# LauraFJulia/TFT_vs_Fund

Measured on AMD Instinct MI355X. Metric: triplet-hypotheses/sec (linearTFT+R,t) at N=200 corresp., higher is better.
Workload: dtype f64; 1 GPU; configs[1]: batch of 10000 synthetic triplets x 200 correspondences, sigma=1px, linearTFT + R_t_from_TFT (LinearTFTPoseEstimation without Reconst), one batch per GPU; batch_per_gpu=10000, correspondences=200, streams=2 (consecutive batches alternate between streams and may overlap), gather=none (1 GPU), failed_triplets=0, warmup_steps_run=2560

## Files before the change

tft_vs_fund_amd/csrc/pose_common.h:

```cpp
#pragma once
#include "wave.h"
#include "small_la.h"
#include "wave_eig.h"
#include "row_eig.h"
#include "wave_qr.h"

namespace tff {

constexpr int FLAG_RECONST = 1;
constexpr int FLAG_JACOBI = 2;
constexpr int FLAG_STAGE_LDS = 4;
constexpr int FLAG_ONLY_RETRY = 8;
constexpr int FLAG_DBG_FP_HANDOVER = 64;
constexpr int FLAG_DBG_ADAPTIVE = 32;
constexpr int FLAG_XI_IN_LDS = 128;
constexpr int FLAG_GH_EXACT = 16;

constexpr int ST_OK = 0;
constexpr int ST_TOO_FEW = 1;
constexpr int ST_NONFINITE = 2;
constexpr int ST_NO_POSE = 3;
constexpr int ST_RETRY = 100;

constexpr int DBG_STRIDE = 128;
// ... 445 lines not shown
                L[r][j] = sv * inv[j];
            }
        }
        double z[3];
#pragma unroll
        for (int r = 2; r >= 0; --r) {
            double sum = -L[3][r];
#pragma unroll
            for (int k = r + 1; k < 3; ++k) sum -= L[k][r] * z[k];
            z[r] = sum * inv[r];
        }
        const double d1 = z[2], d2 = R3[0] * z[0] + R3[1] * z[1] + R3[2] * z[2] + R3[3];
        const double d4 = S33 + delta - (L[3][0] * L[3][0] + L[3][1] * L[3][1] + L[3][2] * L[3][2]);
        const double zz = z[0] * z[0] + z[1] * z[1] + z[2] * z[2];
        const double idet = (inv[0] * inv[1]) * (inv[0] * inv[1]) * (inv[2] * inv[2]);
        const double trs = tr3 + 3.0 * delta;
        const double e = trs * trs * idet;
        const double Gp = 4.0 * (1.0 + zz) - d4 * e;
        const double rhs = 2.0 * d4 * e + 2.5e-14 * trs * e * Gp;
        const double dmin2 = fmin(d1 * d1, d2 * d2);
        const bool certain = Gp > 0.0 && dmin2 * Gp * Gp > rhs * rhs * zz;
        all_certain = all_certain && certain;
        score += (int)sgn(d1) + (int)sgn(d2);
    }
    return 2 * wave_sum_i(score) + (wave_any(!all_certain) ? 1 : 0);
}
struct VoteCam { double PB[12], R3[4]; };
struct VoteFactor { double L[4][3], inv[3], d4, z[3], pfloor; };
template <bool KEEP = false, bool CERT = true>
__device__ __forceinline__ void vote_one(const double (&SA)[6], const VoteCam& cam, const double x2, const double y2, int& score, bool& all_certain,
                                         VoteFactor* keep = nullptr) {
    double b0[4], b1[4];
#pragma unroll
    for (int c = 0; c < 4; ++c) { b0[c] = y2 * cam.PB[8 + c] - cam.PB[4 + c]; b1[c] = cam.PB[c] - x2 * cam.PB[8 + c]; }
    double S[4][3];
#pragma unroll
    for (int r = 0; r < 4; ++r)
#pragma unroll
        for (int c = 0; c < 3; ++c) {
            if (c > r) continue;
            double v = b0[r] * b0[c] + b1[r] * b1[c];
            if (r < 3) v += SA[r * (r + 1) / 2 + c];
            S[r][c] = v;
        }
    const double S33 = b0[3] * b0[3] + b1[3] * b1[3];
    const double tr3 = S[0][0] + S[1][1] + S[2][2];
    const double delta = 1e-14 * (tr3 + S33), pfloor = 1e-3 * delta + 1e-300;
    double L[4][3], inv[3];
#pragma unroll
    for (int j = 0; j < 3; ++j) {
        double d = S[j][j] + delta;
#pragma unroll
        for (int k = 0; k < j; ++k) d -= L[j][k] * L[j][k];
        d = fmax(d, pfloor);
        inv[j] = rsqrt_pos(d);
#pragma unroll
        for (int r = j + 1; r < 4; ++r) {
            double sv = S[r][j];
#pragma unroll
            for (int k = 0; k < j; ++k) sv -= L[r][k] * L[j][k];
            L[r][j] = sv * inv[j];
        }
    }
    double z[3];
#pragma unroll
    for (int r = 2; r >= 0; --r) {
        double sum = -L[3][r];
#pragma unroll
        for (int k = r + 1; k < 3; ++k) sum -= L[k][r] * z[k];
        z[r] = sum * inv[r];
    }
    const double d4 = S33 + delta - (L[3][0] * L[3][0] + L[3][1] * L[3][1] + L[3][2] * L[3][2]);
    if constexpr (CERT) {
        const double d1 = z[2], d2 = cam.R3[0] * z[0] + cam.R3[1] * z[1] + cam.R3[2] * z[2] + cam.R3[3];
        const double zz = z[0] * z[0] + z[1] * z[1] + z[2] * z[2];
        const double idet = (inv[0] * inv[1]) * (inv[0] * inv[1]) * (inv[2] * inv[2]);
        const double trs = tr3 + 3.0 * delta;
        const double e = trs * trs * idet;
        const double Gp = 4.0 * (1.0 + zz) - d4 * e;
        const double rhs = 2.0 * d4 * e + 2.5e-14 * trs * e * Gp;
        const double dmin2 = fmin(d1 * d1, d2 * d2);
        const bool certain = Gp > 0.0 && dmin2 * Gp * Gp > rhs * rhs * zz;
        all_certain = all_certain && certain;
        score += (int)sgn(d1) + (int)sgn(d2);
    }
    if constexpr (KEEP) {
#pragma unroll
        for (int r = 0; r < 4; ++r)
#pragma unroll
            for (int c = 0; c < 3; ++c) keep->L[r][c] = (c < r) ? L[r][c] : 0.0;
#pragma unroll
        for (int c = 0; c < 3; ++c) { keep->inv[c] = inv[c]; keep->z[c] = z[c]; }
        keep->d4 = d4;
        keep->pfloor = pfloor;
    }
}
__device__ __forceinline__ bool dlt_from_vote(const VoteFactor& f, double (&X)[4]) {
    double L[4][4], inv[4];
#pragma unroll
    for (int r = 0; r < 4; ++r)
#pragma unroll
        for (int c = 0; c < 4; ++c) L[r][c] = (c < r) ? f.L[r][c] : 0.0;
    inv[0] = f.inv[0]; inv[1] = f.inv[1]; inv[2] = f.inv[2];
    inv[3] = rsqrt_pos(fmax(f.d4, f.pfloor));
    const double nn0 = 1.0 + (f.z[0] * f.z[0] + f.z[1] * f.z[1] + f.z[2] * f.z[2]);
    const double r0 = rsqrt(nn0);
    const bool fin = nn0 <= 1e300;
    X[0] = fin ? f.z[0] * r0 : 0.5; X[1] = fin ? f.z[1] * r0 : 0.5; X[2] = fin ? f.z[2] * r0 : 0.5; X[3] = fin ? r0 : 0.5;
    bool conv;
    chol_invit<4>(L, inv, X, 40, &conv);
    return conv;
}
template <bool CAM1_IN_REGISTERS>
__device__ __attribute__((noinline)) int tri_vote_fast2(PoseLds* w, const double* pts, int N, int view, const double* camB0, const double* Rt0,
                                                        const double* camB1, const double* Rt1) {
    const int lane = lane_id();
    double PA[12];
    VoteCam c0, c1r;
    load_uniform12(w->Pfin[0], PA);
    load_uniform12(camB0, c0.PB);
#pragma unroll
    for (int c = 0; c < 4; ++c) c0.R3[c] = wave_uniform(Rt0[8 + c]);
    if constexpr (CAM1_IN_REGISTERS) {
#pragma unroll
        for (int c = 0; c < 12; ++c) c1r.PB[c] = camB1[c];
#pragma unroll
        for (int c = 0; c < 4; ++c) c1r.R3[c] = Rt1[8 + c];
    }
    int score0 = 0, score1 = 0;
    bool certain0 = true, certain1 = true;
    Pt6 pnext = load_pt(pts, (lane < N) ? lane : 0);
#pragma unroll 1
    for (int i = lane; i < N; i += WAVE) {
        const Pt6 p = pnext;
        if (i + WAVE < N) pnext = load_pt(pts, i + WAVE);
        const double x1 = p.v[0], y1 = p.v[1], x2 = (view == 1) ? p.v[2] : p.v[4], y2 = (view == 1) ? p.v[3] : p.v[5];
        double a0[3], a1[3], SA[6];
#pragma unroll
        for (int c = 0; c < 3; ++c) { a0[c] = y1 * PA[8 + c] - PA[4 + c]; a1[c] = PA[c] - x1 * PA[8 + c]; }
#pragma unroll
        for (int r = 0; r < 3; ++r)
#pragma unroll
            for (int c = 0; c <= r; ++c) SA[r * (r + 1) / 2 + c] = a0[r] * a0[c] + a1[r] * a1[c];
        vote_one(SA, c0, x2, y2, score0, certain0);
        if constexpr (CAM1_IN_REGISTERS) {
            vote_one(SA, c1r, x2, y2, score1, certain1);
        } else {
            VoteCam c1;
            const double* pb = camB1 + opaque_int(0);
            const double* pr = Rt1 + opaque_int(0);
#pragma unroll
            for (int c = 0; c < 12; ++c) c1.PB[c] = pb[c];
#pragma unroll
            for (int c = 0; c < 4; ++c) c1.R3[c] = pr[8 + c];
            vote_one(SA, c1, x2, y2, score1, certain1);
        }
    }
    const int r0 = 2 * wave_sum_i(score0) + (wave_any(!certain0) ? 1 : 0), r1 = 2 * wave_sum_i(score1) + (wave_any(!certain1) ? 1 : 0);
    return (int)(((unsigned)r1 << 16) | ((unsigned)r0 & 0xffffu));
}
__device__ __attribute__((noinline)) int tri_vote_exact(PoseLds* w, const double* pts, int N, int view, const double* camB, const double* Rt) {
    const int lane = lane_id();
    typedef const double (&cam_ref)[12];
    cam_ref PA = *reinterpret_cast<const double(*)[12]>(w->Pfin[0]);
    cam_ref PB = *reinterpret_cast<const double(*)[12]>(camB);
    double R3[4];
#pragma unroll
// ... 243 lines not shown
```

tft_vs_fund_amd/csrc/small_la.h:

```cpp
#pragma once
#include "wave.h"

namespace tff {

struct Mat3 { double m[3][3]; };

__device__ __forceinline__ double sgn(double x) { return (x > 0.0) ? 1.0 : ((x < 0.0) ? -1.0 : 0.0); }

__device__ __forceinline__ Mat3 mat3_mul(const Mat3& a, const Mat3& b) {
    Mat3 c;
#pragma unroll
    for (int i = 0; i < 3; ++i)
#pragma unroll
        for (int j = 0; j < 3; ++j) c.m[i][j] = a.m[i][0] * b.m[0][j] + a.m[i][1] * b.m[1][j] + a.m[i][2] * b.m[2][j];
    return c;
}
__device__ __forceinline__ Mat3 mat3_T(const Mat3& a) {
    Mat3 c;
#pragma unroll
    for (int i = 0; i < 3; ++i)
#pragma unroll
        for (int j = 0; j < 3; ++j) c.m[i][j] = a.m[j][i];
    return c;
}
__device__ __forceinline__ double mat3_det(const Mat3& a) {
    return a.m[0][0] * (a.m[1][1] * a.m[2][2] - a.m[1][2] * a.m[2][1])
         - a.m[0][1] * (a.m[1][0] * a.m[2][2] - a.m[1][2] * a.m[2][0])
         + a.m[0][2] * (a.m[1][0] * a.m[2][1] - a.m[1][1] * a.m[2][0]);
}
__device__ __forceinline__ Mat3 mat3_inv(const Mat3& a) {
    Mat3 c;
    c.m[0][0] = a.m[1][1] * a.m[2][2] - a.m[1][2] * a.m[2][1];
    c.m[0][1] = a.m[0][2] * a.m[2][1] - a.m[0][1] * a.m[2][2];
    c.m[0][2] = a.m[0][1] * a.m[1][2] - a.m[0][2] * a.m[1][1];
    c.m[1][0] = a.m[1][2] * a.m[2][0] - a.m[1][0] * a.m[2][2];
    c.m[1][1] = a.m[0][0] * a.m[2][2] - a.m[0][2] * a.m[2][0];
    c.m[1][2] = a.m[0][2] * a.m[1][0] - a.m[0][0] * a.m[1][2];
    c.m[2][0] = a.m[1][0] * a.m[2][1] - a.m[1][1] * a.m[2][0];
    c.m[2][1] = a.m[0][1] * a.m[2][0] - a.m[0][0] * a.m[2][1];
    c.m[2][2] = a.m[0][0] * a.m[1][1] - a.m[0][1] * a.m[1][0];
    const double id = 1.0 / (a.m[0][0] * c.m[0][0] + a.m[0][1] * c.m[1][0] + a.m[0][2] * c.m[2][0]);
#pragma unroll
    for (int i = 0; i < 3; ++i)
#pragma unroll
        for (int j = 0; j < 3; ++j) c.m[i][j] *= id;
    return c;
}
__device__ __forceinline__ void cross3(const double* a, const double* b, double* c) {
    c[0] = a[1] * b[2] - a[2] * b[1];
    c[1] = a[2] * b[0] - a[0] * b[2];
    c[2] = a[0] * b[1] - a[1] * b[0];
}

__device__ __forceinline__ double det4(const double (&m)[4][4]) {
    const double s0 = m[0][0] * m[1][1] - m[1][0] * m[0][1], s1 = m[0][0] * m[1][2] - m[1][0] * m[0][2];
    const double s2 = m[0][0] * m[1][3] - m[1][0] * m[0][3], s3 = m[0][1] * m[1][2] - m[1][1] * m[0][2];
    const double s4 = m[0][1] * m[1][3] - m[1][1] * m[0][3], s5 = m[0][2] * m[1][3] - m[1][2] * m[0][3];
    const double c5 = m[2][2] * m[3][3] - m[3][2] * m[2][3], c4 = m[2][1] * m[3][3] - m[3][1] * m[2][3];
    const double c3 = m[2][1] * m[3][2] - m[3][1] * m[2][2], c2 = m[2][0] * m[3][3] - m[3][0] * m[2][3];
    const double c1 = m[2][0] * m[3][2] - m[3][0] * m[2][2], c0 = m[2][0] * m[3][1] - m[3][0] * m[2][1];
    return s0 * c5 - s1 * c4 + s2 * c3 + s3 * c2 - s4 * c1 + s5 * c0;
}

template <int n>
__device__ __forceinline__ int chol_invit(const double (&L)[n][n], const double (&inv)[n], double (&x)[n], const int maxit, bool* converged) {
    bool conv = false;
    double rprev2 = 1.0;
    int it = 0;
#pragma clang loop unroll(disable)
    for (; it < maxit;) {
        double y[n];
#pragma unroll
        for (int i = 0; i < n; ++i) {
            double s = x[i];
#pragma unroll
            for (int k = 0; k < i; ++k) s -= L[i][k] * y[k];
            y[i] = s * inv[i];
        }
#pragma unroll
        for (int i = n - 1; i >= 0; --i) {
            double s = y[i];
#pragma unroll
            for (int k = i + 1; k < n; ++k) s -= L[k][i] * y[k];
            y[i] = s * inv[i];
        }
        double nn = 0.0, dot = 0.0;
#pragma unroll
        for (int i = 0; i < n; ++i) { nn += y[i] * y[i]; dot += y[i] * x[i]; }
        const double rn = rsqrt(nn);
        const double sg = (dot < 0.0) ? -rn : rn;
// ... 401 lines not shown
```

tft_vs_fund_amd/csrc/tft_kernel.h:

```cpp
#pragma once
#include "pose_common.h"

namespace tff {

struct LinearTftArgs {
    const double* corresp;
    const double* calm;
    long calm_stride;
    long B;
    int N;
    int flags;
    double* Rt2;
    double* Rt3;
    double* T;
    double* reconst;
    int* iter;
    int* status;
    double* dbg;
    const int* sample_idx;
    double* init_p;
    double* init_x;
    double* spill;
    long spill_stride;
    int sample_ns;
    const double* pre;
    int* retry_list;
    int* retry_count;
    int* retry_zero;
    const long* offsets;
    const int* rlist;
    const int* rrange;
    int stage_upto;
};

constexpr int EIG_MAXIT = 300;
constexpr int RETRY_HINT_SHIFT = 28;
constexpr int RETRY_INDEX_MASK = (1 << RETRY_HINT_SHIFT) - 1;

__device__ __forceinline__ int ragged_n(const long* offsets, const long b) { return opaque_int(wave_uniform_i((int)(offsets[b + 1] - offsets[b]))); }
__device__ __forceinline__ int ragged_flags(const LinearTftArgs& a, const int n) {
    return opaque_int(n <= a.stage_upto ? (a.flags | FLAG_STAGE_LDS) : (a.flags & ~FLAG_STAGE_LDS));
}
template <bool RAGGED>
__device__ __forceinline__ void ragged_nan_outputs(const LinearTftArgs& a, const long b, const long rb, const int N) {
    if constexpr (RAGGED) wave_nan_outputs(a.Rt2 + b * 12, a.Rt3 + b * 12, a.T + b * 27, a.reconst ? a.reconst + 3 * rb : nullptr, 0, N);
    else wave_nan_outputs(a.Rt2, a.Rt3, a.T, a.reconst, b, N);
}

__device__ __forceinline__ void cvec(const double* a, const double* b, double (&c)[4]) {
    c[0] = a[0] * b[0] + a[1] * b[1];
    c[1] = -(a[0] * b[2] + a[2] * b[0]);
    c[2] = -(a[1] * b[2] + a[2] * b[1]);
    c[3] = a[2] * b[2];
}
__device__ __forceinline__ int hht_index(int i, int ip) {
    const int a = (i < ip) ? i : ip, b = (i < ip) ? ip : i;
    return (a == 0) ? b : ((a == 1) ? 2 + b : 5);
}
__device__ __forceinline__ double bilinear44(const double* M, const double (&c3)[4], const double (&c2)[4]) {
    double acc = 0.0;
#pragma unroll
    for (int p = 0; p < 4; ++p)
        acc += c3[p] * (M[4 * p] * c2[0] + M[4 * p + 1] * c2[1] + M[4 * p + 2] * c2[2] + M[4 * p + 3] * c2[3]);
    return acc;
}

__device__ inline void accumulate_moments(PoseLds* w, const double* pts, int N) {
    const int lane = lane_id();
    const double s1 = w->nrm[0], ox1 = w->nrm[1], oy1 = w->nrm[2];
    const double s2 = w->nrm[3], ox2 = w->nrm[4], oy2 = w->nrm[5];
    const double s3 = w->nrm[6], ox3 = w->nrm[7], oy3 = w->nrm[8];
#pragma unroll 1
    for (int pass = 0; pass < 3; ++pass) {
        double acc[32];
#pragma unroll
        for (int k = 0; k < 32; ++k) acc[k] = 0.0;
        for (int i = lane; i < N; i += WAVE) {
            const Pt6 p = load_pt(pts, i);
            const double x1 = s1 * p.v[0] + ox1, y1 = s1 * p.v[1] + oy1;
            const double x2 = s2 * p.v[2] + ox2, y2 = s2 * p.v[3] + oy2;
            const double x3 = s3 * p.v[4] + ox3, y3 = s3 * p.v[5] + oy3;
            const double q2[4] = {1.0, x2, y2, x2 * x2 + y2 * y2};
            const double q3[4] = {1.0, x3, y3, x3 * x3 + y3 * y3};
            const double pa = (pass == 0) ? x1 * x1 : ((pass == 1) ? x1 : y1);
            const double pb = (pass == 0) ? x1 * y1 : ((pass == 1) ? y1 * y1 : 1.0);
#pragma unroll
            for (int b = 0; b < 4; ++b)
#pragma unroll
                for (int c = 0; c < 4; ++c) {
                    const double wv = q3[b] * q2[c];
                    acc[4 * b + c] += pa * wv;
                    acc[16 + 4 * b + c] += pb * wv;
                }
        }
        const double tot = wave_reduce_scatter<32>(acc);
        if ((lane & 1) == 0) w->mom[32 * pass + reduce32_index(lane)] = tot;
    }
    wave_sync();
}

__device__ __forceinline__ void ctc_entry(int j, int jp, double& sign, int& idx) {
    const int a = (j < jp) ? j : jp, b = (j < jp) ? jp : j;
    if (b < 2) { sign = (a == b) ? 1.0 : 0.0; idx = 0; }
    else if (a < 2) { sign = -1.0; idx = 1 + a; }
    else { sign = 1.0; idx = 3; }
}
__device__ __forceinline__ void gram_row27(const double* mom, int r, double (&g)[27], double& diag) {
    const int i = r / 9, k = (r % 9) / 3, j = r % 3;
    double s2[3], s3[3];
    int i2[3], i3[3];
#pragma unroll
    for (int q = 0; q < 3; ++q) { ctc_entry(j, q, s2[q], i2[q]); ctc_entry(k, q, s3[q], i3[q]); }
#pragma unroll
    for (int ip = 0; ip < 3; ++ip) {
        const double* M = mom + 16 * hht_index(i, ip);
#pragma unroll
        for (int kp = 0; kp < 3; ++kp)
#pragma unroll
            for (int jp = 0; jp < 3; ++jp) g[jp + 3 * kp + 9 * ip] = s2[jp] * s3[kp] * M[4 * i3[kp] + i2[jp]];
    }
    diag = 0.0;
#pragma unroll
    for (int c = 0; c < 27; ++c) diag = (c == r) ? g[c] : diag;
}

__device__ __forceinline__ void frame_of(const double* e, double* Q) {
    const double a0 = fabs(e[0]), a1 = fabs(e[1]), a2 = fabs(e[2]);
    double ax[3] = {0.0, 0.0, 0.0};
    if (a0 <= a1 && a0 <= a2) ax[0] = 1.0; else if (a1 <= a2) ax[1] = 1.0; else ax[2] = 1.0;
    double q1[3], q2[3];
    cross3(e, ax, q1);
    const double n1 = rsqrt(q1[0] * q1[0] + q1[1] * q1[1] + q1[2] * q1[2]);
    q1[0] *= n1; q1[1] *= n1; q1[2] *= n1;
    cross3(e, q1, q2);
    const double n2 = rsqrt(q2[0] * q2[0] + q2[1] * q2[1] + q2[2] * q2[2]);
#pragma unroll
    for (int r = 0; r < 3; ++r) { Q[3 * r] = e[r]; Q[3 * r + 1] = q1[r]; Q[3 * r + 2] = q2[r] * n2; }
}

__device__ __forceinline__ void up_factors(const double* Q, int m, double (&a2)[3], double (&a3)[3]) {
    const int jj = (m < 3) ? 0 : m - 2, kk = (m < 3) ? m : 0;
#pragma unroll
    for (int q = 0; q < 3; ++q) { a2[q] = Q[3 * q + jj]; a3[q] = Q[9 + 3 * q + kk]; }
}

__device__ inline void tft_system_qr(const double* pts, const int N, const double* nrm, double* Rl) {
    const int lane = lane_id();
    for (int e = lane; e < 27 * 27; e += WAVE) Rl[e] = 0.0;
    wave_sync();
    const int col = (lane < 27) ? lane : 0, ci = col / 9, ck = (col % 9) / 3, cj = col % 3;
#pragma unroll 1
    for (int base = 0; base < N; base += 7) {
        double a[28];
#pragma unroll
        for (int q = 0; q < 7; ++q) {
            const int i = base + q;
            const Pt6 p = premap(load_pt(pts, (i < N) ? i : 0), nrm);
            const double h = (i < N && lane < 27) ? ((ci == 0) ? p.v[0] : (ci == 1) ? p.v[1] : 1.0) : 0.0;
            const double c2x = (cj == 0) ? 1.0 : (cj == 1) ? 0.0 : -p.v[2], c2y = (cj == 0) ? 0.0 : (cj == 1) ? 1.0 : -p.v[3];
            const double c3x = (ck == 0) ? 1.0 : (ck == 1) ? 0.0 : -p.v[4], c3y = (ck == 0) ? 0.0 : (ck == 1) ? 1.0 : -p.v[5];
            const double hx = h * c3x, hy = h * c3y;
            a[4 * q + 0] = hx * c2x; a[4 * q + 1] = hx * c2y; a[4 * q + 2] = hy * c2x; a[4 * q + 3] = hy * c2y;
        }
        wave_qr_cols_append<27, 28>(a, Rl);
    }
}

template <bool JAC, int G>
__device__ inline bool linear_tft_middle(PoseLds* w, JacobiLds* jw, const double* pts, int N, bool want_P, double* dbg, const int hint = 0) {
    static_assert(!JAC || G == 64, "the exact solver works on whole wavefronts");
    using Grp = Group<G>;
    const int lane = Grp::lane();
    const int wl = Grp::index() * G;
    int it1 = 0, it2 = 0;
    bool ok = true;
    {
        double x;
        if (JAC) {
            tft_system_qr(pts, N, w->nrm, jw->A);
            phase_stamp(dbg, 3, wl);
            double g[27];
            wave_qr_rows_from_lds<27>(jw->A, g);
            x = wave_qr_min_rsv<27>(g, jw->A, w->Lp, w->Lp, (hint & 1) ? 0 : EIG_MAXIT, &it1);
            if (it1 >= 1000) {
                if (lane < 27) w->t[lane] = x;
                wave_sync();
                tft_system_qr(pts, N, w->nrm, jw->A);
                x = (lane < 27) ? w->t[lane] : 0.0;
            }
            it1 += 10000;
        } else {
            double r2, risk;
            if constexpr (G == 64) {
                const int p = opaque_lane_int(lane & 15);
                const bool hi = p < 11;
                double ga[27], gb[27], g0[16], da, db;
                gram_row27(w->mom, p, ga, da);
                gram_row27(w->mom, hi ? 16 + p : 0, gb, db);
#pragma unroll
                for (int c = 0; c < 16; ++c) g0[c] = ga[c];
#pragma unroll
                for (int c = 0; c < 27; ++c) gb[c] = hi ? gb[c] : 0.0;
                phase_stamp(dbg, 3, wl);
                x = row_min_eigvec<27>(g0, gb, da, hi ? db : 0.0, w->Lp, EIG_MAXIT, &it1, &r2, false, 0.0, 0.0, &risk);
            } else {
                double g[27], diag;
                gram_row27(w->mom, (lane < 27) ? lane : 0, g, diag);
                phase_stamp(dbg, 3, wl);
                x = wave_min_eigvec_reg<27, G>(g, diag, w->Lp, EIG_MAXIT, &it1, &r2, false, 0.0, &risk);
            }
            ok = ok && eig_converged(r2) && risk == 0.0;
        }
        if (lane < 27) w->t[lane] = x;
        wave_sync();
    }
    if (dbg && lane < 27) dbg[lane] = w->t[lane];
    phase_stamp(dbg, 4, wl);
    ok = epipoles_from_tensor<G, JAC>(w->t, w->nullv, w->epi, false) && ok;
    phase_stamp(dbg, 5, wl);
    if (dbg && lane < 6) dbg[27 + lane] = w->epi[lane];
    if (lane == 0) frame_of(w->epi, w->Q);
    if (lane == 1) frame_of(w->epi + 3, w->Q + 9);
    wave_sync();
    if (JAC) {
        double* Bm = w->Lp;
        if (lane < 27) {
// ... 230 lines not shown
```

tft_vs_fund_amd/csrc/tft_rows_kernel.h:

```cpp
#pragma once
#include "tft_kernel.h"
#include "tft_moments_kernel.h"

namespace tff {

constexpr int ROW_TRIPLETS = 4;
constexpr int ROWL = 16;

struct RowRt {
    double T1[28];
    double T2[28];
    double nullv[18];
    double mats[28];
    double Ein[18];
    double cand[2][21];
    double P[4][12];
    double candRt[4][12];
    double Rt[2][12];
    double Pfin[3][12];
};
constexpr int ROW_OV_DOUBLES = 380;
static_assert(sizeof(RowRt) <= ROW_OV_DOUBLES * sizeof(double), "overlay");
struct RowLds {
    double mom[96];
    double nrm[9];
    double calm[27];
    double t[27];
    double epi[6];
    double Q[18];
    double tp[15];
    double pa[18];
    double ov[ROW_OV_DOUBLES];
};
constexpr int ROW_LDS_DOUBLES = (int)(sizeof(RowLds) / sizeof(double));
static_assert(ROW_LDS_DOUBLES % 2 == 0, "16-byte row stride");
inline size_t rows_lds_bytes() { return (size_t)ROW_TRIPLETS * sizeof(RowLds); }
inline unsigned rows_grid(long B) { const long g = (B + ROW_TRIPLETS - 1) / ROW_TRIPLETS; return (unsigned)(g > 0 ? g : 1); }

__device__ __forceinline__ int rows_p() { return lane_id() & 15; }

struct RowSrc { const double* pts; const int* idx; int ns; bool sampled; };
__device__ __forceinline__ Pt6 rows_load(const RowSrc& s, const int i) {
    if (s.sampled) {
        int k = s.idx[i];
        k = (k >= 0 && k < s.ns) ? k : 0;
        return load_pt(s.pts, k);
    }
    return load_pt(s.pts, i);
}

__device__ __forceinline__ void rows_stamp(double* dbg, const int slot) {
    if (dbg) {
        const long long t = shader_clock();
        if (rows_p() == 0) dbg[80 + slot] = (double)t;
    }
}


__device__ __forceinline__ void rows_centroids(const RowSrc& s, const int N, double (&c)[6]) {
    const int p = rows_p();
    double sm[6] = {0, 0, 0, 0, 0, 0};
#pragma unroll 1
    for (int i0 = 0; i0 < N; i0 += 4 * ROWL) {
        Pt6 q[4];
#pragma unroll
        for (int u = 0; u < 4; ++u) { const int i = i0 + ROWL * u + p; q[u] = rows_load(s, (i < N) ? i : 0); }
#pragma unroll
        for (int u = 0; u < 4; ++u) {
            const bool have = i0 + ROWL * u + p < N;
#pragma unroll
            for (int k = 0; k < 6; ++k) sm[k] += have ? q[u].v[k] : 0.0;
        }
    }
#pragma unroll
    for (int k = 0; k < 6; ++k) c[k] = row_sum16(sm[k]) / (double)N;
}

__device__ __forceinline__ void rows_distances_moments(const RowSrc& s, const int N, const double (&c)[6], double* nrm, double (&nr)[9], double* mom) {
    const int p = rows_p();
    const int slot = p >> 1;
    const bool odd = (p & 1) != 0;
    double acc[48];
#pragma unroll
    for (int k = 0; k < 48; ++k) acc[k] = 0.0;
    double dA = 0.0, dB = 0.0;
    auto body = [&](const Pt6& q, double& r2_out) {
        const double x1 = q.v[0] - c[0], y1 = q.v[1] - c[1];
        const double x2 = q.v[2] - c[2], y2 = q.v[3] - c[3];
        const double x3 = q.v[4] - c[4], y3 = q.v[5] - c[5];
        const double r1 = x1 * x1 + y1 * y1, r2 = x2 * x2 + y2 * y2, r3 = x3 * x3 + y3 * y3;
        dA += sqrt_nonneg(odd ? r3 : r1);
        r2_out = r2;
        const double q2[4] = {1.0, x2, y2, r2};
        const double q3[4] = {1.0, x3, y3, r3};
        const double pa = odd ? y1 * y1 : x1 * x1, pb = odd ? y1 : x1 * y1, pc = odd ? 1.0 : x1;
#pragma unroll
        for (int b = 0; b < 4; ++b)
#pragma unroll
            for (int cc = 0; cc < 4; ++cc) {
                const double wv = q3[b] * q2[cc];
                acc[4 * b + cc] += pa * wv;
                acc[16 + 4 * b + cc] += pb * wv;
                acc[32 + 4 * b + cc] += pc * wv;
            }
    };
    constexpr int STEP = ROWL / 2;
    Pt6 pe = rows_load(s, (slot < N) ? slot : 0);
    Pt6 po = rows_load(s, (slot + STEP < N) ? slot + STEP : 0);
#pragma unroll 1
    for (int i = slot; i < N; i += 2 * STEP) {
        const Pt6 q = pe;
        if (i + 2 * STEP < N) pe = rows_load(s, i + 2 * STEP);
        double r2a, r2b = 0.0;
        body(q, r2a);
        if (i + STEP < N) {
            const Pt6 r = po;
            if (i + 3 * STEP < N) po = rows_load(s, i + 3 * STEP);
            body(r, r2b);
        }
        dB += sqrt_nonneg(odd ? r2b : r2a);
    }
    const double d1 = row_sum16(odd ? 0.0 : dA), d3 = row_sum16(odd ? dA : 0.0), d2 = row_sum16(dB);
    const double r2c = sqrt(2.0);
    const double dd[3] = {d1, d2, d3};
#pragma unroll
    for (int v = 0; v < 3; ++v) {
        const double norm0 = dd[v] / (double)N;
        nr[3 * v + 0] = r2c / norm0;
        nr[3 * v + 1] = -r2c * c[2 * v] / norm0;
        nr[3 * v + 2] = -r2c * c[2 * v + 1] / norm0;
    }
    if (p < 9) {
        double mine = nr[0];
#pragma unroll
        for (int k = 1; k < 9; ++k) mine = (p == k) ? nr[k] : mine;
        nrm[p] = mine;
    }
#pragma unroll
    for (int i = 0; i < 24; ++i) acc[i] = halve_sum<8>(acc[i], acc[i + 24]);
#pragma unroll
    for (int i = 0; i < 12; ++i) acc[i] = halve_sum<4>(acc[i], acc[i + 12]);
#pragma unroll
    for (int i = 0; i < 6; ++i) acc[i] = halve_sum<2>(acc[i], acc[i + 6]);
    const int base = 6 * ((p >> 1) & 1) + 12 * ((p >> 2) & 1) + 24 * ((p >> 3) & 1);
    const double s1 = nr[0], s2 = nr[3], s3 = nr[6];
#pragma unroll
// ... 80 lines not shown
            if (r2 <= 1e-26) { res = 0.0; done = true; }
            else if (it >= 2 && r2 < 0.25 * rprev2 && r2 * r2 < 1e-26 * rprev2) { res = 0.0; done = true; }
            else if (!(r2 == r2) || it >= maxit) { res = (r2 == r2) ? r2 : 1.0; done = true; }
            if (it >= 2 && r2 > 1e-30) { rk_r2 = r2; rk_rp = rprev2; rk_nn = nn; }
            rprev2 = r2;
        }
        if (!wave_any(!done)) break;
    }
    *iters = it;
    *resid2 = res;
    if (gram_risk) {
        const double num = 4.0 * rk_nn * rk_r2 * rk_rp;
        const double d = rk_rp - rk_r2;
        const double den = (rk_r2 < rk_rp) ? d * d : 0.0;
        *gram_risk = (tr * tr * num < gram_risk_limit2 * den) ? 0.0 : 1.0;
    }
}

template <class MatFn>
__device__ __forceinline__ void rows_transform_tft_inverse(const double* to, double* tn, double* mats, MatFn matrix_of) {
    const int p = rows_p();
    if (p < 3) {
        Mat3 M = matrix_of(p);
        if (p > 0) M = mat3_inv(M);
#pragma unroll
        for (int r = 0; r < 3; ++r)
#pragma unroll
            for (int c = 0; c < 3; ++c) mats[9 * p + 3 * r + c] = M.m[r][c];
    }
    wave_sync();
    double val[2];
#pragma unroll
    for (int h = 0; h < 2; ++h) {
        const int e = 16 * h + p;
        const bool have = e < 27;
        const int ee = have ? e : 0;
        const int i = ee / 9, k = (ee % 9) / 3, j = ee % 3;
        const double m0 = mats[i], m1 = mats[3 + i], m2 = mats[6 + i];
        double v = 0.0;
#pragma unroll
        for (int c = 0; c < 3; ++c)
#pragma unroll
            for (int d = 0; d < 3; ++d) {
                const double mix = m0 * to[c + 3 * d] + m1 * to[c + 3 * d + 9] + m2 * to[c + 3 * d + 18];
                v += mats[9 + 3 * j + c] * mix * mats[18 + 3 * k + d];
            }
        val[h] = have ? v : 0.0;
    }
    const double nn = row_sum16(val[0] * val[0] + val[1] * val[1]);
    const double rs = rsqrt(nn);
    wave_sync();
    tn[p] = val[0] * rs;
    if (p < 11) tn[16 + p] = val[1] * rs;
    wave_sync();
}

__device__ __forceinline__ bool rows_linear_tft_middle(RowLds* w, double* dbg, const bool want_P = false) {
    const int p = opaque_lane_int(rows_p());
    bool ok = true;
    int it1 = 0, it2 = 0;
    {
        const bool hi = p < 11;
        double ga[27], gb[27], g0[16], da, db, r2, risk, x0, x1;
        gram_row27(w->mom, p, ga, da);
        gram_row27(w->mom, hi ? 16 + p : 0, gb, db);
#pragma unroll
        for (int c = 0; c < 16; ++c) g0[c] = ga[c];
#pragma unroll
        for (int c = 0; c < 27; ++c) gb[c] = hi ? gb[c] : 0.0;
        rows_stamp(dbg, 3);
        rows_min_eigvec<27>(g0, gb, da, hi ? db : 0.0, w->ov, EIG_MAXIT, &it1, &r2, false, 0.0, 0.0, &risk, x0, x1);
        ok = ok && eig_converged(r2) && risk == 0.0;
        wave_sync();
        w->t[p] = x0;
        if (hi) w->t[16 + p] = x1;
        wave_sync();
    }
    if (dbg) { dbg[p] = w->t[p]; if (p < 11) dbg[16 + p] = w->t[16 + p]; }
    rows_stamp(dbg, 4);
    const bool eok = epipoles_from_tensor<16, false>(w->t, w->ov, w->epi, false);
    ok = !row_any(!eok) && ok;
    rows_stamp(dbg, 5);
    if (dbg && p < 6) dbg[27 + p] = w->epi[p];
    if (p == 0) frame_of(w->epi, w->Q);
    if (p == 1) frame_of(w->epi + 3, w->Q + 9);
    wave_sync();
    double* Gp = w->ov;
#pragma unroll 1
    for (int e = p; e < 120; e += ROWL) {
        int a = (int)((sqrtf(8.0f * (float)e + 1.0f) - 1.0f) * 0.5f);
        while (tri_index(a + 1, 0) <= e) ++a;
        while (tri_index(a, 0) > e) --a;
        const int b = e - tri_index(a, 0);
        double a2[3], a3[3], b2[3], b3[3], c2[4], c3[4];
        up_factors(w->Q, a % 5, a2, a3);
        up_factors(w->Q, b % 5, b2, b3);
        cvec(a2, b2, c2);
        cvec(a3, b3, c3);
        Gp[e] = bilinear44(w->mom + 16 * hht_index(a / 5, b / 5), c3, c2);
    }
    wave_sync();
    rows_stamp(dbg, 6);
    {
        double g[15], none[1] = {0.0}, diag = 0.0, x0, x1, r2, risk;
        const bool have = p < 15;
        const int r = have ? p : 0;
#pragma unroll
        for (int c = 0; c < 15; ++c) { g[c] = (c <= r && have) ? Gp[tri_index(r, c)] : 0.0; diag = (c == r) ? g[c] : diag; }
        double tp0 = 0.0;
        if (have) {
            const int i = r / 5, m = r % 5, jj = (m < 3) ? 0 : m - 2, kk = (m < 3) ? m : 0;
#pragma unroll
            for (int k = 0; k < 3; ++k)
#pragma unroll
                for (int j = 0; j < 3; ++j) tp0 += w->Q[3 * j + jj] * w->Q[9 + 3 * k + kk] * w->t[j + 3 * k + 9 * i];
        }
        wave_sync();
        rows_min_eigvec<15>(g, none, diag, 0.0, w->ov, EIG_MAXIT, &it2, &r2, true, tp0, 0.0, &risk, x0, x1);
        ok = ok && eig_converged(r2) && risk == 0.0;
        if (have) w->tp[p] = x0;
        wave_sync();
    }
    rows_stamp(dbg, 7);
    {
        double tv[2];
#pragma unroll
        for (int h = 0; h < 2; ++h) {
            const int e = (16 * h + p < 27) ? 16 * h + p : 0;
            const int i = e / 9, k = (e % 9) / 3, j = e % 3;
            double acc = 0.0;
#pragma unroll
            for (int m = 0; m < 5; ++m) {
                const int jj = (m < 3) ? 0 : m - 2, kk = (m < 3) ? m : 0;
                acc += w->Q[3 * j + jj] * w->Q[9 + 3 * k + kk] * w->tp[5 * i + m];
            }
            tv[h] = acc;
        }
        wave_sync();
        w->t[p] = tv[0];
        if (p < 11) w->t[16 + p] = tv[1];
        wave_sync();
    }
    if (dbg) {
        dbg[33 + p] = w->t[p];
        if (p < 11) dbg[33 + 16 + p] = w->t[16 + p];
        if (p == 0) { dbg[69] = (double)it1; dbg[70] = (double)it2; }
    }
    if (want_P) {
        if (p < 3) {
            const int i = p;
            const double* e21 = w->epi; const double* e31 = w->epi + 3;
            double ai[3], bi[3];
            for (int j = 0; j < 3; ++j) ai[j] = w->t[j + 9 * i] * e31[0] + w->t[j + 3 + 9 * i] * e31[1] + w->t[j + 6 + 9 * i] * e31[2];
            const double ae = ai[0] * e21[0] + ai[1] * e21[1] + ai[2] * e21[2];
            for (int k = 0; k < 3; ++k) {
                const double tte = w->t[3 * k + 9 * i] * e21[0] + w->t[1 + 3 * k + 9 * i] * e21[1] + w->t[2 + 3 * k + 9 * i] * e21[2];
                bi[k] = e31[k] * ae - tte;
            }
            const double be = bi[0] * e31[0] + bi[1] * e31[1] + bi[2] * e31[2];
            const double n21 = e21[0] * e21[0] + e21[1] * e21[1] + e21[2] * e21[2];
            const double n31 = e31[0] * e31[0] + e31[1] * e31[1] + e31[2] * e31[2];
            const double c = -(ae + be) / (n21 + n31);
            for (int j = 0; j < 3; ++j) { w->pa[3 * i + j] = ai[j] + c * e21[j]; w->pa[9 + 3 * i + j] = bi[j] + c * e31[j]; }
        }
        wave_sync();
    }
    return ok;
}

__device__ __forceinline__ void rows_recover_prepare(RowLds* w, RowRt* rt);
template <bool EXACT = false>
__device__ __forceinline__ bool rows_rt_prepare(RowLds* w, RowRt* rt, double* dbg) {
    const int p = rows_p();
    rows_transform_tft_inverse(rt->T1, rt->T2, rt->mats, [w](int v) { return load_K(w->calm, v); });
    const bool eok = epipoles_from_tensor<16, EXACT>(rt->T2, rt->nullv, w->epi, true);
    const bool ok = !row_any(!eok);
    if (p < 2) {
        const double* e21 = w->epi; const double* e31 = w->epi + 3;
        Mat3 M;
#pragma unroll
        for (int i = 0; i < 3; ++i)
#pragma unroll
// ... 82 lines not shown
    double snum = 0.0, sden = 0.0;
    bool sconv = true;
#pragma unroll 1
    for (int sweep = 0; sweep < 2; ++sweep) {
        ++sweeps;
        const int start = (sweep == 0) ? 0 : ROWL;
        Pt6 pnext = rows_load(s, (start + p < N) ? start + p : 0);
#pragma unroll 1
        for (int i0 = start; i0 < N; i0 += ROWL) {
            const Pt6 q = pnext;
            const bool have = i0 + p < N;
            pnext = rows_load(s, (i0 + ROWL + p < N) ? i0 + ROWL + p : 0);
            const double x1 = q.v[0], y1 = q.v[1];
            double a0[3], a1[3], SA[6];
#pragma unroll
            for (int c = 0; c < 3; ++c) { a0[c] = y1 * PA[8 + c] - PA[4 + c]; a1[c] = PA[c] - x1 * PA[8 + c]; }
#pragma unroll
            for (int rr = 0; rr < 3; ++rr)
#pragma unroll
                for (int c = 0; c <= rr; ++c) SA[rr * (rr + 1) / 2 + c] = a0[rr] * a0[c] + a1[rr] * a1[c];
            const bool first = sweep == 0 && i0 == 0;
#pragma unroll
            for (int cc = 0; cc < 2; ++cc) {
                const int call = 1 - cc;
                const double x2 = (call == 0) ? q.v[2] : q.v[4], y2 = (call == 0) ? q.v[3] : q.v[5];
                VoteFactor fA, fB;
                if (evalA) {
                    VoteCam cam;
                    const int off = opaque_lane_int(offA[call]);
                    const double* pb = rt->P[0] + off;
                    const double* pr = rt->candRt[0] + off;
#pragma unroll
                    for (int c = 0; c < 12; ++c) cam.PB[c] = pb[c];
#pragma unroll
                    for (int c = 0; c < 4; ++c) cam.R3[c] = pr[8 + c];
                    int term = 0;
                    bool cert = true;
                    if (SPEC && call == 0 && !first) vote_one<true, false>(SA, cam, x2, y2, term, cert, &fA);
                    else if (SPEC && call == 0) vote_one<true>(SA, cam, x2, y2, term, cert, &fA);
                    else vote_one(SA, cam, x2, y2, term, cert);
                    scA[call] += have ? term : 0;
                    certA[call] = certA[call] && (cert || !have);
                }
                if (evalB[call]) {
                    VoteCam cam;
                    const int off = opaque_lane_int(offB[call]);
                    const double* pb = rt->P[0] + off;
                    const double* pr = rt->candRt[0] + off;
#pragma unroll
                    for (int c = 0; c < 12; ++c) cam.PB[c] = pb[c];
#pragma unroll
                    for (int c = 0; c < 4; ++c) cam.R3[c] = pr[8 + c];
                    int term = 0;
                    bool cert = true;
                    if (SPEC && call == 0 && first) vote_one<true>(SA, cam, x2, y2, term, cert, &fB);
                    else vote_one(SA, cam, x2, y2, term, cert);
                    scB[call] += have ? term : 0;
                    certB[call] = certB[call] && (cert || !have);
                }
                if (first) {
                    const bool v0 = row_any(have && certA[call] && scA[call] != 2), v1 = row_any(have && certA[call] && scA[call] != -2);
                    const bool b0 = row_any(have && certB[call] && scB[call] != 2), b1 = row_any(have && certB[call] && scB[call] != -2);
                    const bool mixA = v0 && v1, mixB = b0 && b1;
                    const bool single = !all4 && (mixA != mixB);
                    main1[call] = single && mixA;
                    if (main1[call]) {
                        const int ts = scA[call]; scA[call] = scB[call]; scB[call] = ts;
                        const bool tc = certA[call]; certA[call] = certB[call]; certB[call] = tc;
                        offA[call] = 12 + 24 * call; offB[call] = 24 * call;
                        if (SPEC && call == 0) fA = fB;
                    }
                    rowB[call] = !single;
                    evalB[call] = wave_any(!single);
                    fullB[call] = evalB[call];
                }
                if (SPEC && call == 0 && evalA) {
                    double X[4];
                    const bool conv = dlt_from_vote(fA, X);
                    sconv = sconv && (conv || !have);
                    if (!first) {
                        const double* pr = rt->candRt[0] + opaque_lane_int(offA[0]);
                        const double s4 = sgn(X[3]);
                        const double d1 = X[2] * s4, d2 = (pr[8] * X[0] + pr[9] * X[1] + pr[10] * X[2] + pr[11] * X[3]) * s4;
                        scA[0] += have ? (int)sgn(d1) + (int)sgn(d2) : 0;
                        certA[0] = certA[0] && (conv || !have);
                    }
                    const double iw = 1.0 / X[3];
                    const double X0 = X[0] * iw, X1 = X[1] * iw, X2 = X[2] * iw;
                    const double* ax = rt->P[0] + opaque_lane_int(offA[1]);
                    double X3[3], u3[3];
#pragma unroll
                    for (int r = 0; r < 3; ++r) { X3[r] = ax[4 * r] * X0 + ax[4 * r + 1] * X1 + ax[4 * r + 2] * X2; u3[r] = ax[4 * r + 3]; }
                    const double p3[3] = {q.v[4], q.v[5], 1.0};
                    double c1[3], c2[3];
                    cross3(p3, X3, c1);
                    cross3(p3, u3, c2);
                    snum += have ? c1[0] * c2[0] + c1[1] * c2[1] + c1[2] * c2[2] : 0.0;
                    sden += have ? c2[0] * c2[0] + c2[1] * c2[1] + c2[2] * c2[2] : 0.0;
                }
            }
        }
        if (sweep == 1) break;
        bool again = false;
#pragma unroll
        for (int call = 0; call < 2; ++call) {
            const int tA = (int)row_sum16((double)scA[call]);
            const bool mine = !rowB[call] && tA != 2 * N && tA != -2 * N;
            rowB[call] = rowB[call] || mine;
            const bool need = wave_any(!fullB[call] && tA != 2 * N && tA != -2 * N);
            evalB[call] = need;
            fullB[call] = fullB[call] || need;
            again = again || need;
        }
        evalA = false;
        if (!again) break;
    }
    bool ok = true;
#pragma unroll
    for (int call = 0; call < 2; ++call) {
        const int tA = (int)row_sum16((double)scA[call]);
        const int tBsum = (int)row_sum16((double)scB[call]);
        const int tB = (fullB[call] && rowB[call]) ? tBsum : 0;
        const bool badA = row_any(!certA[call]), badB = row_any(!certB[call]);
        ok = ok && !badA && (!(fullB[call] && rowB[call]) || !badB);
        if (cert_out) {
            cert_out[2 * call] = main1[call] ? !badB : !badA;
            cert_out[2 * call + 1] = main1[call] ? !badA : !badB;
        }
        sc[call][0] = main1[call] ? tB : tA;
        sc[call][1] = main1[call] ? tA : tB;
    }
    if constexpr (SPEC) {
        scale->num = row_sum16(snum);
        scale->den = row_sum16(sden);
        scale->conv = !row_any(!sconv);
        scale->main1[0] = main1[0];
        scale->main1[1] = main1[1];
    }
    if (sweeps_out) *sweeps_out = sweeps + (fullB[0] ? 16 : 0) + (fullB[1] ? 32 : 0);
    return ok;
}

template <int MODE, bool EXACT = false>
__device__ __forceinline__ bool rows_tri_pass(const RowSrc& s, const int N, const double* camA, const double* camB, const double* aux,
                                              double* out, double& num_out, double& den_out) {
    const int p = rows_p();
    double PAr[12], PBr[12], AXr[12];
    if (!EXACT) {
#pragma unroll
        for (int c = 0; c < 12; ++c) { PAr[c] = camA[c]; PBr[c] = camB[c]; AXr[c] = aux[c]; }
    }
    typedef const double (&cam_ref)[12];
    cam_ref PA = EXACT ? *reinterpret_cast<const double(*)[12]>(camA) : PAr;
    cam_ref PB = EXACT ? *reinterpret_cast<const double(*)[12]>(camB) : PBr;
    cam_ref AX = EXACT ? *reinterpret_cast<const double(*)[12]>(aux) : AXr;
    bool all_conv = true;
    double num = 0.0, den = 0.0;
    Pt6 pnext = rows_load(s, (p < N) ? p : 0);
#pragma unroll 1
    for (int i = p; i < N; i += ROWL) {
        const Pt6 q = pnext;
        if (i + ROWL < N) pnext = rows_load(s, i + ROWL);
        double X[4];
        const bool conv = dlt_point<EXACT, EXACT>(PA, PB, AX, camA, camB, aux, MODE == TRI_RECONST, q.v[0], q.v[1], q.v[2], q.v[3], q.v[4], q.v[5], X);
        all_conv = all_conv && conv;
        const double iw = 1.0 / X[3];
        const double X0 = X[0] * iw, X1 = X[1] * iw, X2 = X[2] * iw;
// ... 322 lines not shown
```

Baseline: 95.52 million triplet-hypotheses/s.

## Replace index arithmetic with packed constexpr lookup tables and integer sign helper

Several unrelated micro-optimisations are bundled. Index computations in the Gram-row and Gp-fill loops (ctc_entry, hht_index, and the sqrt-based triangular index inversion) are replaced with constexpr bit-packed lookup words. The 27-way diagonal selection becomes a direct moment load, the sign scoring uses an integer sgn helper instead of a double-to-int conversion, and the centroid loop gets a bounds-check-free main body. Each change trims a little scalar ALU work, and the packed tables add some bit manipulation and correctness risk in the encodings.

```diff
diff --git a/tft_vs_fund_amd/csrc/pose_common.h b/tft_vs_fund_amd/csrc/pose_common.h
--- a/tft_vs_fund_amd/csrc/pose_common.h
+++ b/tft_vs_fund_amd/csrc/pose_common.h
@@ -551,7 +551,7 @@
         const double dmin2 = fmin(d1 * d1, d2 * d2);
         const bool certain = Gp > 0.0 && dmin2 * Gp * Gp > rhs * rhs * zz;
         all_certain = all_certain && certain;
-        score += (int)sgn(d1) + (int)sgn(d2);
+        score += sgn_i(d1) + sgn_i(d2);
     }
     if constexpr (KEEP) {
 #pragma unroll
diff --git a/tft_vs_fund_amd/csrc/small_la.h b/tft_vs_fund_amd/csrc/small_la.h
--- a/tft_vs_fund_amd/csrc/small_la.h
+++ b/tft_vs_fund_amd/csrc/small_la.h
@@ -6,6 +6,7 @@
 struct Mat3 { double m[3][3]; };
 
 __device__ __forceinline__ double sgn(double x) { return (x > 0.0) ? 1.0 : ((x < 0.0) ? -1.0 : 0.0); }
+__device__ __forceinline__ int sgn_i(double x) { return (int)(x > 0.0) - (int)(x < 0.0); }
 
 __device__ __forceinline__ Mat3 mat3_mul(const Mat3& a, const Mat3& b) {
     Mat3 c;
diff --git a/tft_vs_fund_amd/csrc/tft_kernel.h b/tft_vs_fund_amd/csrc/tft_kernel.h
--- a/tft_vs_fund_amd/csrc/tft_kernel.h
+++ b/tft_vs_fund_amd/csrc/tft_kernel.h
@@ -105,23 +105,46 @@
     else if (a < 2) { sign = -1.0; idx = 1 + a; }
     else { sign = 1.0; idx = 3; }
 }
+constexpr unsigned ctc_row_word(const int j) {
+    unsigned w = 0;
+    for (int q = 0; q < 3; ++q) {
+        const int a = (j < q) ? j : q, b = (j < q) ? q : j;
+        const int idx = (b < 2) ? 0 : ((a < 2) ? 1 + a : 3);
+        const int sg = (b < 2) ? ((a == b) ? 1 : 0) : ((a < 2) ? -1 : 1);
+        w |= (unsigned)idx << (2 * q) | (unsigned)(sg + 1) << (8 + 2 * q);
+    }
+    return w;
+}
+__device__ __forceinline__ void ctc_row(const int j, double (&sign)[3], int (&idx)[3]) {
+    constexpr unsigned long long ROWS = (unsigned long long)ctc_row_word(0) | (unsigned long long)ctc_row_word(1) << 16 | (unsigned long long)ctc_row_word(2) << 32;
+    const unsigned w = (unsigned)(ROWS >> (16 * j));
+#pragma unroll
+    for (int q = 0; q < 3; ++q) {
+        idx[q] = (int)((w >> (2 * q)) & 3u);
+        sign[q] = (double)((int)((w >> (8 + 2 * q)) & 3u) - 1);
+    }
+}
+__device__ __forceinline__ unsigned hht_row_word(const int i) {
+    constexpr unsigned R0 = 0u | 1u << 3 | 2u << 6, R1 = 1u | 3u << 3 | 4u << 6, R2 = 2u | 4u << 3 | 5u << 6;
+    constexpr unsigned long long ROWS = (unsigned long long)R0 | (unsigned long long)R1 << 16 | (unsigned long long)R2 << 32;
+    return (unsigned)(ROWS >> (16 * i));
+}
 __device__ __forceinline__ void gram_row27(const double* mom, int r, double (&g)[27], double& diag) {
     const int i = r / 9, k = (r % 9) / 3, j = r % 3;
     double s2[3], s3[3];
     int i2[3], i3[3];
-#pragma unroll
-    for (int q = 0; q < 3; ++q) { ctc_entry(j, q, s2[q], i2[q]); ctc_entry(k, q, s3[q], i3[q]); }
+    ctc_row(j, s2, i2);
+    ctc_row(k, s3, i3);
+    const unsigned hw = hht_row_word(i);
 #pragma unroll
     for (int ip = 0; ip < 3; ++ip) {
-        const double* M = mom + 16 * hht_index(i, ip);
+        const double* M = mom + 16 * (int)((hw >> (3 * ip)) & 7u);
 #pragma unroll
         for (int kp = 0; kp < 3; ++kp)
 #pragma unroll
             for (int jp = 0; jp < 3; ++jp) g[jp + 3 * kp + 9 * ip] = s2[jp] * s3[kp] * M[4 * i3[kp] + i2[jp]];
     }
-    diag = 0.0;
-#pragma unroll
-    for (int c = 0; c < 27; ++c) diag = (c == r) ? g[c] : diag;
+    diag = mom[16 * (int)((hw >> (3 * i)) & 7u) + ((k == 2) ? 12 : 0) + ((j == 2) ? 3 : 0)];
 }
 
 __device__ __forceinline__ void frame_of(const double* e, double* Q) {
@@ -138,10 +161,29 @@
     for (int r = 0; r < 3; ++r) { Q[3 * r] = e[r]; Q[3 * r + 1] = q1[r]; Q[3 * r + 2] = q2[r] * n2; }
 }
 
+__device__ __forceinline__ void up_factors_jk(const double* Q, int jj, int kk, double (&a2)[3], double (&a3)[3]) {
+#pragma unroll
+    for (int q = 0; q < 3; ++q) { a2[q] = Q[3 * q + jj]; a3[q] = Q[9 + 3 * q + kk]; }
+}
 __device__ __forceinline__ void up_factors(const double* Q, int m, double (&a2)[3], double (&a3)[3]) {
-    const int jj = (m < 3) ? 0 : m - 2, kk = (m < 3) ? m : 0;
-#pragma unroll
-    for (int q = 0; q < 3; ++q) { a2[q] = Q[3 * q + jj]; a3[q] = Q[9 + 3 * q + kk]; }
+    up_factors_jk(Q, (m < 3) ? 0 : m - 2, (m < 3) ? m : 0, a2, a3);
+}
+struct GpIndexTable { unsigned long long w[16][2]; };
+constexpr GpIndexTable make_gp_index_table() {
+    GpIndexTable t{};
+    for (int p = 0; p < 16; ++p)
+        for (int k = 0; k < 8; ++k) {
+            const int e = p + 16 * k;
+            if (e >= 120) continue;
+            int a = 0;
+            while ((a + 1) * (a + 2) / 2 <= e) ++a;
+            const int b = e - a * (a + 1) / 2;
+            const int ma = a % 5, mb = b % 5, lo = b / 5, hi = a / 5;
+            const unsigned word = (unsigned)((ma < 3) ? 0 : ma - 2) | (unsigned)((ma < 3) ? ma : 0) << 2 | (unsigned)((mb < 3) ? 0 : mb - 2) << 4
+                                  | (unsigned)((mb < 3) ? mb : 0) << 6 | (unsigned)((lo == 0) ? hi : ((lo == 1) ? 2 + hi : 5)) << 8;
+            t.w[p][k >> 2] |= (unsigned long long)word << (16 * (k & 3));
+        }
+    return t;
 }
 
 __device__ inline void tft_system_qr(const double* pts, const int N, const double* nrm, double* Rl) {
diff --git a/tft_vs_fund_amd/csrc/tft_rows_kernel.h b/tft_vs_fund_amd/csrc/tft_rows_kernel.h
--- a/tft_vs_fund_amd/csrc/tft_rows_kernel.h
+++ b/tft_vs_fund_amd/csrc/tft_rows_kernel.h
@@ -60,8 +60,18 @@
 __device__ __forceinline__ void rows_centroids(const RowSrc& s, const int N, double (&c)[6]) {
     const int p = rows_p();
     double sm[6] = {0, 0, 0, 0, 0, 0};
+    int i0 = 0;
 #pragma unroll 1
-    for (int i0 = 0; i0 < N; i0 += 4 * ROWL) {
+    for (; i0 + 4 * ROWL <= N; i0 += 4 * ROWL) {
+        Pt6 q[4];
+#pragma unroll
+        for (int u = 0; u < 4; ++u) q[u] = rows_load(s, i0 + ROWL * u + p);
+#pragma unroll
+        for (int u = 0; u < 4; ++u)
+#pragma unroll
+            for (int k = 0; k < 6; ++k) sm[k] += q[u].v[k];
+    }
+    if (i0 < N) {
         Pt6 q[4];
 #pragma unroll
         for (int u = 0; u < 4; ++u) { const int i = i0 + ROWL * u + p; q[u] = rows_load(s, (i < N) ? i : 0); }
@@ -308,22 +318,21 @@
     ok = !row_any(!eok) && ok;
     rows_stamp(dbg, 5);
     if (dbg && p < 6) dbg[27 + p] = w->epi[p];
-    if (p == 0) frame_of(w->epi, w->Q);
-    if (p == 1) frame_of(w->epi + 3, w->Q + 9);
+    if (p < 2) frame_of(w->epi + 3 * p, w->Q + 9 * p);
     wave_sync();
     double* Gp = w->ov;
+    constexpr GpIndexTable gp_index = make_gp_index_table();
+    const unsigned long long gw0 = gp_index.w[rows_p()][0], gw1 = gp_index.w[rows_p()][1];
+    int trip = 0;
 #pragma unroll 1
-    for (int e = p; e < 120; e += ROWL) {
-        int a = (int)((sqrtf(8.0f * (float)e + 1.0f) - 1.0f) * 0.5f);
-        while (tri_index(a + 1, 0) <= e) ++a;
-        while (tri_index(a, 0) > e) --a;
-        const int b = e - tri_index(a, 0);
+    for (int e = p; e < 120; e += ROWL, ++trip) {
+        const unsigned gw = (unsigned)(((trip < 4) ? gw0 : gw1) >> (16 * (trip & 3)));
         double a2[3], a3[3], b2[3], b3[3], c2[4], c3[4];
-        up_factors(w->Q, a % 5, a2, a3);
-        up_factors(w->Q, b % 5, b2, b3);
+        up_factors_jk(w->Q, (int)(gw & 3u), (int)((gw >> 2) & 3u), a2, a3);
+        up_factors_jk(w->Q, (int)((gw >> 4) & 3u), (int)((gw >> 6) & 3u), b2, b3);
         cvec(a2, b2, c2);
         cvec(a3, b3, c3);
-        Gp[e] = bilinear44(w->mom + 16 * hht_index(a / 5, b / 5), c3, c2);
+        Gp[e] = bilinear44(w->mom + 16 * (int)((gw >> 8) & 7u), c3, c2);
     }
     wave_sync();
     rows_stamp(dbg, 6);
@@ -572,7 +581,7 @@
                         const double* pr = rt->candRt[0] + opaque_lane_int(offA[0]);
                         const double s4 = sgn(X[3]);
                         const double d1 = X[2] * s4, d2 = (pr[8] * X[0] + pr[9] * X[1] + pr[10] * X[2] + pr[11] * X[3]) * s4;
-                        scA[0] += have ? (int)sgn(d1) + (int)sgn(d2) : 0;
+                        scA[0] += have ? sgn_i(d1) + sgn_i(d2) : 0;
                         certA[0] = certA[0] && (conv || !have);
                     }
                     const double iw = 1.0 / X[3];
```

Result: faster. 97.51 million triplet-hypotheses/s (median of 6 runs) (+2.1%).
